# al8n/serf

Measured on NVIDIA H100. Metric: gossip edge-updates/sec @10M nodes, higher is better.
Workload: dtype u32

## Files before the change

### include/serfsim.h

```cpp
#ifndef SERFSIM_H
#define SERFSIM_H

#include <stddef.h>
#include <stdint.h>

#ifdef __cplusplus
extern "C" {
#endif

#define SERFSIM_ABI_VERSION 4u

#define SERFSIM_OK            0
#define SERFSIM_E_INVAL      (-1)
#define SERFSIM_E_NO_DEVICE  (-2)
#define SERFSIM_E_CUDA       (-3)
#define SERFSIM_E_NOMEM      (-4)
#define SERFSIM_E_OVERFLOW   (-5)
#define SERFSIM_E_COMM       (-6)

#define SERFSIM_STATUS_NONE     0u
#define SERFSIM_STATUS_ALIVE    1u
#define SERFSIM_STATUS_LEAVING  2u
#define SERFSIM_STATUS_LEFT     3u
#define SERFSIM_STATUS_FAILED   4u
// ... 122 lines not shown

int serfsim_set_user_events(serfsim_t* h, uint32_t n_events, const uint32_t* content_ids );
int serfsim_event_time       (serfsim_t* h, uint64_t* out );
int serfsim_user_event_seen  (serfsim_t* h, uint32_t event, uint8_t* out );
int serfsim_user_event_ltime (serfsim_t* h, uint32_t event, uint64_t* ltime);
int serfsim_user_event_records(serfsim_t* h, void* out );
int serfsim_user_event_stats (serfsim_t* h, serfsim_uevent_stats_t* out);

int serfsim_set_byzantine  (serfsim_t* h, uint32_t n, const uint32_t* ids , uint32_t delta);
int serfsim_anomaly_flags  (serfsim_t* h, uint8_t* out );
int serfsim_byzantine_stats(serfsim_t* h, serfsim_byz_stats_t* out);

int serfsim_last_step_device_ms(serfsim_t* h, double* ms, uint64_t* kernel_launches);
int serfsim_set_tick_timing(serfsim_t* h, int enabled);
int serfsim_tick_times(serfsim_t* h, uint32_t first_tick, uint32_t n, float* ms_out);

size_t serfsim_comm_blob_size(void);
int    serfsim_comm_export (serfsim_t* h, void* blob);
int    serfsim_comm_connect(serfsim_t* h, const void* blobs );
typedef void (*serfsim_barrier_fn)(void* user);
typedef void (*serfsim_allreduce_u64_fn)(void* user, uint64_t* buf, uint32_t n);
int    serfsim_comm_set_hooks(serfsim_t* h, serfsim_barrier_fn barrier, serfsim_allreduce_u64_fn allreduce, void* user);
int    serfsim_comm_loopback(serfsim_t* h);

#define SERFSIM_WIRE_LEAVE     1u
#define SERFSIM_WIRE_JOIN      2u
#define SERFSIM_WIRE_PUSH_PULL 3u
typedef struct { uint32_t type , prune ; uint64_t ltime, id; } serfsim_wire_intent_t;
typedef struct {
  uint64_t ltime, event_ltime, query_ltime;
// ... 41 lines not shown
```

### serf_b200/csrc/serfsim.cu

```cuda
#include <algorithm>
#include <cmath>
#include <cstdio>
#include <cstdlib>
#include <cstring>
#include <string>
#include <unordered_set>
#include <vector>

#include "../../include/serfsim.h"
#include "tick_kernel.cuh"
#include "wire.cuh"

using namespace sfs;

namespace {

thread_local std::string g_err;

int fail(int code, const std::string& msg) { g_err = msg; return code; }

#define CU(call)                                                                              \
  do {                                                                                        \
    cudaError_t e_ = (call);                                                                  \
    if (e_ != cudaSuccess)                                                                    \
// ... 71 lines not shown
  const uint4** d_peer_snap_rec = nullptr;
  const u64** d_peer_snap_node = nullptr;
  u8* d_hot[2] = {nullptr, nullptr};
  u8* d_hot_static = nullptr;
  u32* d_node_due = nullptr;
  u32* d_carry = nullptr;
  u32* d_tile_due = nullptr;
  u32* d_sched = nullptr;
  u32 n_tiles = 0;
  u32* d_rowptr = nullptr;
  u32* d_col = nullptr;
  u32 *d_ev_node = nullptr, *d_ev_op = nullptr, *d_ev_slot = nullptr;
  size_t ev_cap = 0;
  u64* d_trace = nullptr;
  u32* d_kinds = nullptr;
  u32* d_ones = nullptr;
  u32 trace_cap = 0;
  u32* d_overflow = nullptr;
  u32* pin_overflow = nullptr;
  u32* d_subj = nullptr;
  u64* d_scratch = nullptr;
  void* d_stage = nullptr;
  UeTable ue_table{};
  uint4* d_ue_state = nullptr;
  u32* d_ue_inbox[2] = {nullptr, nullptr};
  u32* d_ue_ltime = nullptr;
  wire::UeWire ue_wire{};
  u8* d_ue_entries = nullptr;
  u64* d_ue_totals = nullptr;
  u32 ue_injected = 0;
// ... 67 lines not shown
  std::vector<cudaEvent_t> tick_ev;
  std::vector<cudaEvent_t> mid_ev;
};

namespace {

int slot_of(const serfsim* h, u32 node) {
  for (u32 s = 0; s < h->R; ++s) if (h->subj[s] == node) return (int)s;
  return -1;
}

int ensure_trace(serfsim* h, u32 need) {
  if (need <= h->trace_cap) return 0;
  u32 cap = std::max<u32>(1024, h->trace_cap);
  while (cap < need) cap *= 2;
  u64* nt = nullptr; u32* nk = nullptr; u64* ng = nullptr;
  const bool sharded = h->cfg.world_size > 1;
  CU(cudaMalloc(&nt, (size_t)cap * 8 * sizeof(u64)));
  CU(cudaMalloc(&nk, ((size_t)cap + 1) * 4 * sizeof(u32)));
  CU(cudaMemsetAsync(nt, 0, (size_t)cap * 8 * sizeof(u64), h->stream));
  CU(cudaMemsetAsync(nk, 0, ((size_t)cap + 1) * 4 * sizeof(u32), h->stream));
  if (sharded) { CU(cudaMalloc(&ng, (size_t)cap * 8 * sizeof(u64))); CU(cudaMemsetAsync(ng, 0, (size_t)cap * 8 * sizeof(u64), h->stream)); }
  if (h->d_trace) {
    CU(cudaMemcpyAsync(nt, h->d_trace, (size_t)h->trace_cap * 8 * sizeof(u64), cudaMemcpyDeviceToDevice, h->stream));
    CU(cudaMemcpyAsync(nk, h->d_kinds, ((size_t)h->trace_cap + 1) * 4 * sizeof(u32), cudaMemcpyDeviceToDevice, h->stream));
    if (sharded) CU(cudaMemcpyAsync(ng, h->d_grow, (size_t)h->trace_cap * 8 * sizeof(u64), cudaMemcpyDeviceToDevice, h->stream));
    CU(cudaStreamSynchronize(h->stream));
    cudaFree(h->d_trace); cudaFree(h->d_kinds); cudaFree(h->d_grow);
  }
  h->d_trace = nt; h->d_kinds = nk; h->d_grow = ng; h->trace_cap = cap;
  return 0;
}

int upload_ops(serfsim* h) {
  if (!h->ops_dirty) return 0;
  std::stable_sort(h->ops.begin(), h->ops.end(), [](const HostOp& a, const HostOp& b) { return a.tick != b.tick ? a.tick < b.tick : a.seq < b.seq; });
  const size_t n = h->ops.size();
  if (n > h->ev_cap) {
    size_t cap = std::max<size_t>(1024, h->ev_cap);
    while (cap < n) cap *= 2;
    if (h->d_ev_node) { cudaFree(h->d_ev_node); cudaFree(h->d_ev_op); cudaFree(h->d_ev_slot); }
    CU(cudaMalloc(&h->d_ev_node, cap * 4)); CU(cudaMalloc(&h->d_ev_op, cap * 4)); CU(cudaMalloc(&h->d_ev_slot, cap * 4));
    h->ev_cap = cap;
  }
  if (n) {
    std::vector<u32> a(n), b(n), c(n);
    for (size_t i = 0; i < n; ++i) { a[i] = h->ops[i].node; b[i] = h->ops[i].op; c[i] = h->ops[i].slot; }
    CU(cudaMemcpyAsync(h->d_ev_node, a.data(), n * 4, cudaMemcpyHostToDevice, h->stream));
    CU(cudaMemcpyAsync(h->d_ev_op, b.data(), n * 4, cudaMemcpyHostToDevice, h->stream));
    CU(cudaMemcpyAsync(h->d_ev_slot, c.data(), n * 4, cudaMemcpyHostToDevice, h->stream));
    CU(cudaStreamSynchronize(h->stream));
  }
  h->ops_dirty = false;
  return 0;
}

bool future_ops(const serfsim* h, u32 after_tick) {
  return !h->ops.empty() && h->ops.back().tick > after_tick;
}

int launch_ticks(serfsim* h, u32 n) {
  if (!h->has_topo) return fail(SERFSIM_E_INVAL, "serfsim_step: no topology set");
  if (h->cfg.world_size > 1 && !h->connected) return fail(SERFSIM_E_COMM, "serfsim_step: world_size > 1 but serfsim_comm_connect was not called");
  int rc = upload_ops(h);
  if (rc) return rc;
  rc = ensure_trace(h, h->tick + n + 1);
  if (rc) return rc;
  if (!h->timing_open) { CU(cudaEventRecord(h->ev0, h->stream)); h->timing_open = true; h->last_launches = 0; h->launch_log.clear(); h->launch_log_first = h->tick; }
  const bool sharded = h->cfg.world_size > 1;
  const u64* grow = sharded ? h->d_grow : h->d_trace;
  for (u32 i = 0; i < n; ++i) {
    const u32 t = h->tick;
    const u64 launches_before = h->last_launches;
// ... 10 lines not shown
    p.fanout = h->cfg.fanout; p.probe_every = h->cfg.probe_interval_ticks; p.tick = t;
    p.down_mask = (~h->up_mask) & ((1u << h->R) - 1);
    h->ever_down |= p.down_mask;
    p.seed_lo = (u32)h->cfg.seed; p.seed_hi = (u32)(h->cfg.seed >> 32); p.ev_begin = eb; p.ev_end = ee;
    p.rules = h->rules;
    for (u32 s = 0; s < h->R; ++s) p.subj[s] = h->subj[s];
    p.rec = h->d_rec; p.qword = h->d_qword; p.inbox_rd = h->d_inbox[(t & 1) ^ 1]; p.inbox_wr = h->d_inbox[t & 1];
    p.node_state = h->d_node; p.busy = h->d_busy; p.watch = h->d_watch; p.row_ptr = h->d_rowptr; p.col = h->d_col;
    p.ev_node = h->d_ev_node; p.ev_op = h->d_ev_op; p.ev_slot = h->d_ev_slot;
    p.row = h->d_trace + (size_t)t * 8;
    p.kinds_prev = h->d_kinds + (size_t)t * 4;
    p.kinds_cur = h->d_kinds + ((size_t)t + 1) * 4;
    p.overflow = h->d_overflow;
    p.hot_rd = h->d_hot[(t & 1) ^ 1]; p.hot_wr = h->d_hot[t & 1];
    p.stage_col_bytes = h->stage_col_bytes;
    p.reap_now = (h->cfg.reap_interval_ticks && ((t + 1) % h->cfg.reap_interval_ticks) == 0) ? 1u : 0u;
    p.tombstone_ticks = h->cfg.tombstone_timeout_ticks; p.reconnect_ticks = h->cfg.reconnect_timeout_ticks; p.intent_ticks = h->cfg.recent_intent_timeout_ticks;
    p.stride = h->stride; p.n_tiles = h->n_tiles; p.tiles_per_cta = (h->n_tiles + h->grid - 1) / h->grid;
    p.force_all = (h->cfg.trace != 0) || h->no_skip || p.reap_now;
    p.compact = h->compact ? 1u : 0u;
    p.dedup = h->dedup ? 1u : 0u;
    p.udeg = h->udeg; p.ahead = h->ahead;
    p.tile_due = h->d_tile_due; p.node_due = h->d_node_due; p.hot_static = h->d_hot_static; p.sched = h->d_sched;
    p.sleep_on = (h->no_skip || h->byz_on) ? 0u : 1u;
    p.pp_every = (u32)std::max(0, h->cfg.push_pull_interval_ticks); p.reap_every = h->cfg.reap_interval_ticks;
    p.host_idle_until = h->d_pin_ctl + 2;
    const u32 xpar = h->xepoch & 1;
    p.world = (u32)h->cfg.world_size; p.rank = (u32)h->cfg.rank; p.shard_size = h->shard_size; p.win_cap = h->win_cap;
    p.win_data = h->d_peer_data[xpar]; p.send_count = h->d_send_count;
    p.peer_ctrl = h->d_peer_ctrl; p.stamp = h->xepoch + 1; p.xpar = xpar; p.loopback = h->loopback ? 1u : 0u;
    p.fuse_publish = (sharded && !h->byz_on && !getenv("SERFSIM_NO_FUSE")) ? 1u : 0u;
// ... 23 lines not shown
    if (h->ue_table.n) {
      UeParams u{};
      u.n_local = h->count; u.first = h->first; u.n_global = h->N; u.R = h->R; u.fanout = h->cfg.fanout; u.tick = t;
      u.seed_lo = p.seed_lo; u.seed_hi = p.seed_hi; u.limit = h->rules.limit; u.ev_begin = eb; u.ev_end = ee;
      u.table = h->ue_table; u.state = h->d_ue_state; u.inbox_rd = h->d_ue_inbox[(t & 1) ^ 1]; u.inbox_wr = h->d_ue_inbox[t & 1];
      u.ltime = h->d_ue_ltime; u.node_state = h->d_node; u.busy = h->d_busy; u.row_ptr = h->d_rowptr; u.col = h->d_col;
      u.ev_node = h->d_ev_node; u.ev_op = h->d_ev_op; u.ev_slot = h->d_ev_slot;
      u.row = p.row; u.totals = h->d_ue_totals; u.overflow = h->d_overflow; u.sched = h->d_sched;
      u.world = (u32)h->cfg.world_size; u.rank = (u32)h->cfg.rank; u.shard_size = h->shard_size; u.win_cap = h->win_cap;
      u.win_data = h->d_peer_data[h->xepoch & 1]; u.send_count = h->d_send_count;
      u.gate = gate; u.gate.evaluate = 1u;
      launch_uevent(u, h->cfg.trace != 0, h->stream);
      h->last_launches++;
    }
    const bool sv_ok = h->sv && h->R > 1 && h->R < 32 && !h->cfg.trace && p.sleep_on && !h->byz_on;
    const bool pass_tick = sv_ok && !sharded && ee == eb && !p.reap_now && t + 1 < CARRY_TICKS;
    const bool dual = sv_ok && sharded && __builtin_popcount(h->ever_down) == 1;
    if (pass_tick || dual) {
      const bool all = ee > eb || p.reap_now;
      p.views_host = all ? 0xffffffffu : h->ever_down;
      p.sv_mode = h->sv == 2 ? SV_CHECK : SV_GENERAL;
      p.sv_slot = h->ever_down ? (u32)__builtin_ctz(h->ever_down) : 0u; p.sv_R = h->R;
    }
    if (pass_tick && h->sv == 1) {
      p.sv_mode = SV_PASS; p.carry = h->d_carry;
      p.tiles_per_cta = (h->n_tiles + h->grid_sv - 1) / h->grid_sv;
      for (u32 s0 = 0; s0 < h->R; ++s0) {
        TickParams q = p;
        q.gate.evaluate = s0 == 0 ? p.gate.evaluate : 0u; q.sv_wshift = s0; q.sv_slot = s0;
        q.rec = p.rec + 2 * (size_t)s0 * h->stride; q.qword = p.qword + (size_t)s0 * h->stride;
        q.inbox_rd = p.inbox_rd + (size_t)s0 * h->stride; q.inbox_wr = p.inbox_wr + (size_t)s0 * h->stride;
        q.subj[0] = p.subj[s0]; q.down_mask = (p.down_mask >> s0) & 1u;
        launch_tick_pass(q, h->grid_sv, h->stream);
        h->last_launches++;
      }
    } else {
      launch_tick(p, h->cfg.trace != 0, h->grid, h->stream);
      h->last_launches++;
    }
    if (dual && h->sv == 1) {
      TickParams q = p;
      const u32 s0 = p.sv_slot;
      q.sv_mode = SV_SINGLE; q.gate.evaluate = 0u; q.sv_wshift = s0;
      q.rec = p.rec + 2 * (size_t)s0 * h->stride; q.qword = p.qword + (size_t)s0 * h->stride;
// ... 184 lines not shown
  CU(cudaMemsetAsync(h->d_inbox[1], 0, inbox_bytes, h->stream));
  CU(cudaStreamSynchronize(h->stream));
  *(volatile u32*)h->pin_overflow = 0;
  ((volatile u32*)h->pin_ctl)[2] = 0;
  CU(cudaMemsetAsync(h->d_busy, 0, h->stride, h->stream));
  CU(cudaMemsetAsync(h->d_qword, 0, (size_t)h->R * h->stride * 4, h->stream));
  CU(cudaMemsetAsync(h->d_hot[0], 0, h->n_tiles, h->stream));
  CU(cudaMemsetAsync(h->d_hot[1], 0, h->n_tiles, h->stream));
  CU(cudaMemsetAsync(h->d_tile_due, 0xff, (size_t)h->n_tiles * sizeof(u32), h->stream));
  CU(cudaMemsetAsync(h->d_node_due, 0xff, (size_t)h->stride * sizeof(u32), h->stream));
  if (h->d_carry) CU(cudaMemsetAsync(h->d_carry, 0, (size_t)h->stride * sizeof(u32), h->stream));
  CU(cudaMemsetAsync(h->d_sched, 0, SCHED_WORDS * sizeof(u32), h->stream));
  if (h->d_trace) {
    CU(cudaMemsetAsync(h->d_trace, 0, (size_t)h->trace_cap * 8 * sizeof(u64), h->stream));
    CU(cudaMemsetAsync(h->d_kinds, 0, ((size_t)h->trace_cap + 1) * 4 * sizeof(u32), h->stream));
  }
  if (h->d_grow) CU(cudaMemsetAsync(h->d_grow, 0, (size_t)h->trace_cap * 8 * sizeof(u64), h->stream));
  CU(cudaMemsetAsync(h->d_runctl, 0, 2 * sizeof(u32), h->stream));
  if (h->d_send_count) CU(cudaMemsetAsync(h->d_send_count, 0, sizeof(u32) * 8, h->stream));
  { int rc = ue_reset(h); if (rc) return rc; }
  if (h->d_anomaly) { CU(cudaMemsetAsync(h->d_anomaly, 0, h->stride, h->stream)); CU(cudaMemsetAsync(h->d_byz_totals, 0, 4 * 8, h->stream)); }
  { int rc = refresh_watchers(h); if (rc) return rc; }
  CU(cudaStreamSynchronize(h->stream));
  return 0;
}

void free_all(serfsim* h) {
  for (void* p : h->ipc_opened) cudaIpcCloseMemHandle(p);
  for (cudaEvent_t e : h->tick_ev) cudaEventDestroy(e);
  cudaFree(h->d_hot_static); cudaFree(h->d_tile_due); cudaFree(h->d_node_due); cudaFree(h->d_carry); cudaFree(h->d_sched);
  cudaFree(h->d_hot[0]); cudaFree(h->d_hot[1]); cudaFree(h->d_busy); cudaFree(h->d_watch); cudaFree(h->d_snap_rec); cudaFree(h->d_snap_node); cudaFree(h->d_peer_snap_rec); cudaFree(h->d_peer_snap_node);
  cudaFree(h->d_qword);
  cudaFree(h->d_rec); cudaFree(h->d_inbox[0]); cudaFree(h->d_inbox[1]); cudaFree(h->d_node); cudaFree(h->d_rowptr); cudaFree(h->d_col);
  cudaFree(h->d_ev_node); cudaFree(h->d_ev_op); cudaFree(h->d_ev_slot); cudaFree(h->d_trace); cudaFree(h->d_kinds); cudaFree(h->d_ones);
  if (h->pin_overflow) cudaFreeHost(h->pin_overflow);
  cudaFree(h->d_subj); cudaFree(h->d_scratch); cudaFree(h->d_stage);
  cudaFree(h->d_byz_ids); cudaFree(h->d_anomaly); cudaFree(h->d_byz_totals); cudaFree(h->d_peer_anomaly);
  cudaFree(h->d_ue_snap); cudaFree(h->d_peer_ue_snap);
  cudaFree(h->d_ue_entries);
  cudaFree(h->d_ue_state); cudaFree(h->d_ue_inbox[0]); cudaFree(h->d_ue_inbox[1]); cudaFree(h->d_ue_ltime); cudaFree(h->d_ue_totals);
  for (int par = 0; par < 2; ++par) { cudaFree(h->d_win_data[par]); cudaFree(h->d_peer_data[par]); }
  cudaFree(h->d_ctrl); cudaFree(h->d_send_count); cudaFree(h->d_peer_ctrl);
  for (auto& b : h->res) { cudaFree(b.d); if (b.copied) cudaEventDestroy(b.copied); }
  if (h->ev_extracted) cudaEventDestroy(h->ev_extracted);
  if (h->copy_stream) cudaStreamDestroy(h->copy_stream);
  if (h->pin_ctl) cudaFreeHost(h->pin_ctl);
  cudaFree(h->d_runctl); cudaFree(h->d_grow);
  if (h->ev0) cudaEventDestroy(h->ev0);
  if (h->ev1) cudaEventDestroy(h->ev1);
// ... 703 lines not shown
}

int serfsim_set_tick_timing(serfsim_t* h, int enabled) {
  if (!h) return fail(SERFSIM_E_INVAL, "null handle");
  h->tick_timing = enabled != 0;
  return 0;
}

int serfsim_tick_times(serfsim_t* h, uint32_t first_tick, uint32_t n, float* ms_out) {
  if (!h || !ms_out) return fail(SERFSIM_E_INVAL, "null argument");
  if (((size_t)first_tick + n) * 2 > h->tick_ev.size()) return fail(SERFSIM_E_INVAL, "tick timing was not enabled for that range");
  CU(cudaStreamSynchronize(h->stream));
  for (u32 i = 0; i < n; ++i) CU(cudaEventElapsedTime(ms_out + i, h->tick_ev[2 * ((size_t)first_tick + i)], h->tick_ev[2 * ((size_t)first_tick + i) + 1]));
  return 0;
}

struct comm_blob { cudaIpcMemHandle_t data[2]; cudaIpcMemHandle_t ctrl; cudaIpcMemHandle_t snap_rec, snap_node, anomaly, ue_snap; u32 win_cap; u32 rank; u32 has_snap; u32 has_ue_snap; unsigned char dev_uuid[16]; };

size_t serfsim_comm_blob_size(void) { return sizeof(comm_blob); }

int serfsim_comm_export(serfsim_t* h, void* blob) {
  if (!h || !blob) return fail(SERFSIM_E_INVAL, "null argument");
  if (h->cfg.world_size < 2) return fail(SERFSIM_E_INVAL, "world_size == 1: nothing to export");
  comm_blob b{};
  for (int par = 0; par < 2; ++par) CU(cudaIpcGetMemHandle(&b.data[par], h->d_win_data[par]));
  CU(cudaIpcGetMemHandle(&b.ctrl, h->d_ctrl));
  CU(cudaIpcGetMemHandle(&b.anomaly, h->d_anomaly));
  if (h->d_ue_snap) { CU(cudaIpcGetMemHandle(&b.ue_snap, h->d_ue_snap)); b.has_ue_snap = 1; }
  b.win_cap = h->win_cap; b.rank = (u32)h->cfg.rank;
#ifndef SERFSIM_EMU
// ... 102 lines not shown
```

### serf_b200/csrc/tick_kernel.cu

```cuda
#include <cstdlib>

#include "tick_kernel.cuh"
#include "byz.cuh"

namespace sfs {

namespace {

constexpr int BLOCK = 256;
#ifndef SFS_MB_R1
#define SFS_MB_R1 3
#endif
#ifndef SFS_MB_R1S
#define SFS_MB_R1S SFS_MB_R1
#endif
#ifndef SFS_MB_RN
#define SFS_MB_RN 1
#endif
constexpr u32 TILE_SHIFT = 8;
constexpr u32 MAX_TILES_PER_CTA = 1024;
static_assert((1u << TILE_SHIFT) == BLOCK, "tile = block");

struct Words { u32 w[8]; };

// ... 278 lines not shown
  x.mL = x.mJ = x.mM = x.qw = 0; x.any = 0; x.mailmask = 0; x.qmask = 0;
  for (u32 s2 = 0; s2 < s_hi; ++s2) {
    const u32 l = kL ? ld_u32_stream(p.inbox_rd + (size_t)(KIND_LEAVE * R + s2) * nl + vl, pol_first) : 0u;
    const u32 j = kJ ? ld_u32_stream(p.inbox_rd + (size_t)(KIND_JOIN * R + s2) * nl + vl, pol_first) : 0u;
    const u32 m = kM ? ld_u32_stream(p.inbox_rd + (size_t)(KIND_ML * R + s2) * nl + vl, pol_first) : 0u;
    const u32 q = p.qword[(size_t)s2 * nl + vl];
    SFS_COUNT(6, 4);
    if (R1 || s2 == x.keep) { x.mL = l; x.mJ = j; x.mM = m; x.qw = q; }
    x.any |= l | j | m;
    x.mailmask |= ((l | j | m) ? 1u : 0u) << s2;
    x.qmask |= (q ? 1u : 0u) << s2;
  }
  if (PASS) x.any |= x.qw | ((due && (carry_of(p, vl) & CARRY_TDUE)) ? 1u : 0u);
  return x;
}
__device__ __forceinline__ bool node_active(const TickParams& p, const Pre& x, bool due) {
  return (x.busy & 7u) != 0 || x.any != 0 || p.reap_now != 0 || (due && (x.busy & 8u) && x.nd <= p.tick);
}

template <int FMAX>
struct Ahead { u64 ns; Words rec; u32 cand[FMAX]; u32 valid; };

__device__ __forceinline__ u32 sleeping_deadline(const Pre& x, bool due) { return (due && (x.busy & 8u)) ? x.nd : NO_DEADLINE; }

#if defined(SFS_COLD_INLINE)
#define SFS_COLD __forceinline__
#elif defined(SERFSIM_EMU)
#define SFS_COLD __attribute__((noinline))
#else
#define SFS_COLD __noinline__
#endif
__device__ SFS_COLD void cold_host_op(Rec& r, u32& clock, u32& sstate, u32 op, bool op_here, bool self, bool up_r, u32 limit) {
// ... 88 lines not shown
      cur = ld_rec256(p.rec + 2 * (size_t)vl, pol_first);
    }
    merge_q(cur, pre.qw);
  };
  if (upfront) { load_node(); load_rec0(); }
  const u32 busy = pre.busy;
  u32 mL = pre.mL, mJ = pre.mJ, mM = pre.mM;
  if (STAGED) { mL = kL ? sv.inL[lt] : 0u; mJ = kJ ? sv.inJ[lt] : 0u; mM = kM ? sv.inM[lt] : 0u; }

  u32 nd = pre.nd;
  if (R1 && due && (busy & 8u)) nd = p.node_due[vl];
  const u32 sleeping = (due && (busy & 8u)) ? nd : NO_DEADLINE;
  bool timers_due = sleeping <= p.tick;
  u32 cr = 0;
  if (PASS && due) { cr = carry_of(p, vl); if (cr & CARRY_SEEN) timers_due = (cr & CARRY_TDUE) != 0; }
  if (!TRACE && !STAGED && !((busy & 7u) != 0 || pre.any != 0 || p.reap_now != 0 || timers_due)) { mind = min(mind, sleeping); if (due && (busy & 8u)) SFS_PROBE(20); return false; }
  if (PASS && !due) cr = carry_of(p, vl);
  if (STAGED && !TRACE && !((busy & 7u) || (mL | mJ | mM) || p.reap_now || timers_due)) { mind = min(mind, sleeping); return false; }
#define SFS_WMASK() ((busy & 4u) ? ((u32)p.watch[vl] >> p.sv_wshift) : 0u)
  const bool ahead = !R1 && !STAGED && ah.valid;
  if (ahead) { ns = ah.ns; row0 = vl * p.udeg; row1 = row0 + p.udeg; }
  else if (!upfront) { load_node(); if (R1) load_rec0(); }

  u32 clock = (u32)ns;
  const bool up_r = (ns & NS_UP) != 0;
  u32 sstate = (u32)(ns >> 40) & 3;
  const u32 deg = row1 - row0;

  u32 op = 0, op_slot = 0;
  if (busy & 2) { u32 slot_tmp = 0; op = cold_find_op(p, v, slot_tmp); op_slot = slot_tmp; }
  bool up_s = up_r;
// ... 235 lines not shown
#pragma unroll
  for (int i = 0; i < 8; ++i) {
    const u32 s = warp_sum((u32)vals[i]);
    if (lane == 0) red[i][wid] = s;
  }
  u64 hs = 0;
  if (TRACE) hs = warp_sum64(c.hash);
  __syncthreads();
  if (threadIdx.x == 0 && dsusp_cta) atomicAdd(reinterpret_cast<unsigned long long*>(p.sched + SCHED_SUSPECTS), (unsigned long long)(long long)dsusp_cta);
  if (threadIdx.x < 8) {
    u64 s = 0;
#pragma unroll
    for (int w = 0; w < BLOCK / 32; ++w) s += red[threadIdx.x][w];
    if (s) {
      if (threadIdx.x < 5) atomicAdd((unsigned long long*)(p.row + threadIdx.x), (unsigned long long)s);
      else atomicAdd(p.kinds_cur + (threadIdx.x - 5), (u32)min(s, (u64)0xffffffffu));
    }
  }
  if (TRACE && lane == 0 && hs) atomicAdd((unsigned long long*)(p.row + 7), (unsigned long long)hs);
  { const u32 vw = __reduce_or_sync(0xffffffffu, c.views); if (lane == 0 && vw) atomicOr(p.sched + SCHED_VIEWS_NEXT, vw); }
  if (PASS && p.sv_slot + 1u < p.sv_R) return;
  __threadfence();
  __syncthreads();
  if (threadIdx.x == 0) last_s = (atomicAdd(p.sched + SCHED_TICKET, 1u) == gridDim.x - 1) ? 1u : 0u;
  __syncthreads();
  if (!last_s) return;
  __threadfence();
  volatile u32* sched = p.sched;
  volatile u64* row = p.row;
  const u64 suspects = *reinterpret_cast<volatile u64*>(p.sched + SCHED_SUSPECTS);
  __shared__ u32 quiet_s;
// ... 51 lines not shown
    const u32 views = (sv_base | p.views_host) & ((1u << p.sv_R) - 1u);
    work = (views >> p.sv_slot) & 1u;
    carry_out = (views >> p.sv_slot) > 1u;
    if (work) SFS_PROBE(21);
    else if (p.sv_slot != 0 && p.sv_slot + 1u < p.sv_R) return;
  } else if (p.sv_mode != SV_OFF) {
    const u32 sv_base = p.tick >= p.sched[SCHED_VIEWS_FROM] ? p.sched[SCHED_VIEWS_NEW] : p.sched[SCHED_VIEWS_OLD];
    const u32 views = (sv_base | p.views_host) & ((1u << p.sv_R) - 1u);
    const bool single = views == (1u << p.sv_slot);
    if (p.sv_mode == SV_SINGLE) { if (!single) return; SFS_PROBE(21); }
    else if (p.sv_mode == SV_GENERAL && single) return;
    if (p.sv_mode == SV_CHECK && (single || p.world == 1)) sv_views = views;
  }
  if (threadIdx.x == 0) dsusp_s = 0;
  Counters c = {};
  const bool kL = p.kinds_prev[KIND_LEAVE] != 0, kJ = p.kinds_prev[KIND_JOIN] != 0, kM = p.kinds_prev[KIND_ML] != 0;
  const u64 pol_first = policy_evict_first(), pol_last = policy_evict_last();
  const int lane = threadIdx.x & 31;
  if (SHARDED && threadIdx.x < (BLOCK / 32) * MAX_WORLD) xs->cnt[threadIdx.x / MAX_WORLD][threadIdx.x % MAX_WORLD] = 0;
  bool wrote_remote = false;
  u32 resv = 0, rlen = 0;

  const u32 prev_msgs = p.kinds_prev[KIND_LEAVE] + p.kinds_prev[KIND_JOIN] + p.kinds_prev[KIND_ML];
  const bool dense_now = prev_msgs >= (p.n_tiles >> 1) + 1;
  const bool all_hot = p.force_all || p.kinds_prev[3] != 0;
  const bool mark = !dense_now;
  const bool saturated = prev_msgs >= (p.n_local >> 1);
  if (dense_now && blockIdx.x == 0 && threadIdx.x == 0) p.kinds_cur[3] = 1;

  const u32 tile0 = blockIdx.x * p.tiles_per_cta;
  const u32 ntile = tile0 < p.n_tiles ? min(p.tiles_per_cta, p.n_tiles - tile0) : 0;
  if (SHARDED && saturated && ntile && (u32)lane < p.world && (u32)lane != p.rank) { resv = atomicAdd(p.send_count + lane, XW_FLUSH); rlen = XW_FLUSH; }
  if (PASS && p.sv_slot != 0) tile_decisions(p, hot_s, tile0, ntile, p.sv_slot + 1u == p.sv_R, work); else scan_tiles(p, hot_s, tile0, ntile, all_hot, PASS);
  __syncthreads();
  if (PASS && !work && p.sv_slot + 1u < p.sv_R) return;
  constexpr u32 GROUP = SHARDED ? 4 : 8;
  __shared__ uint4 act_s[GROUP * BLOCK];
  __shared__ u32 act_n;
  __shared__ u8 pend_s[GROUP];
  __shared__ u16 gt_s[GROUP];
  const bool compact = !TRACE && !saturated && !p.reap_now && p.compact;
  if (compact) {
    u32 i = 0;
// ... 6 lines not shown
      __syncthreads();
      Pre pr[GROUP];
#pragma unroll
      for (u32 g = 0; g < GROUP; ++g) {
        pr[g] = Pre{};
        if (g < ng) {
          const u32 vn = ((tile0 + gt_s[g]) << TILE_SHIFT) + threadIdx.x;
          if (vn < p.n_local) pr[g] = prefetch_node<R1, PASS>(p, vn, kL, kJ, kM, pol_first, PASS && (hot_s[gt_s[g]] & 2u) != 0);
        }
      }
#pragma unroll
      for (u32 g = 0; g < GROUP; ++g) {
        const bool due_g = g < ng && (hot_s[gt_s[g]] & 2u) != 0;
        Pre prg = pr[g];
        if (due_g && (prg.busy & 8u)) prg.nd = p.node_due[((tile0 + gt_s[g]) << TILE_SHIFT) + threadIdx.x];
        const bool act = g < ng && node_active(p, prg, due_g);
        if (due_g) {
          const u32 wm = warp_min(act ? NO_DEADLINE : sleeping_deadline(prg, true));
          if (lane == 0 && wm != NO_DEADLINE) atomicMin(p.tile_due + tile0 + gt_s[g], wm);
          if (!act && (prg.busy & 8u)) SFS_PROBE(20);
        }
        const u32 bal = __ballot_sync(0xffffffffu, act);
        if (bal) {
          u32 base = 0;
          if (lane == 0) base = atomicAdd(&act_n, (u32)__popc(bal));
          base = __shfl_sync(0xffffffffu, base, 0);
          if (act) act_s[base + (u32)__popc(bal & ((1u << lane) - 1u))] =
              make_uint4((g << 8) | threadIdx.x | (pr[g].busy << 16) | ((pr[g].any ? 1u : 0u) << 24), pr[g].mL, pr[g].mJ, pr[g].mM);
        }
      }
      __syncthreads();
// ... 632 lines not shown
```

### serf_b200/csrc/tick_kernel.cuh

```cuda
#pragma once
#include <cuda_runtime.h>

#include "record.cuh"
#include "uevent.cuh"

#if defined(SERFSIM_EMU) && defined(__CUDACC__)
#error "SERFSIM_EMU is the host-only test build of tests/emu (g++); the product is built by nvcc without it"
#endif
#ifndef SERFSIM_EMU
#define SFS_LAUNCH(grid, block, smem, stream, ...) __VA_ARGS__<<<(grid), (block), (smem), (stream)>>>
constexpr int SFS_SMS = 132;
#else
constexpr int SFS_SMS = 1;
#endif
#ifdef SERFSIM_EMU
#define SFS_PROBE(i) (emu::probes[i]++)
#define SFS_COUNT(i, n) (emu::probes[i] += (n))
#else
#define SFS_PROBE(i) ((void)0)
#define SFS_COUNT(i, n) ((void)0)
#endif

namespace sfs {

// ... 60 lines not shown
  Gate gate;
  u32 udeg;
  u32* tile_due;
  u32* node_due;
  const u8* hot_static;
  u32* sched;
  u32 sleep_on;
  u32 pp_every, reap_every;
  u32* const* peer_ctrl; u32 stamp, xpar, loopback, fuse_publish;
  u32 shard_inv, xcap;
  u32 sv_wshift;
  u32 sv_mode, views_host, sv_slot, sv_R;
  u32 ahead;
  u32* host_idle_until;
  u32* carry;
};
constexpr u32 SCHED_TICKET = 0, SCHED_IDLE_UNTIL = 1, SCHED_UE_ACTIVITY = 2, SCHED_AWAKE = 3, SCHED_SUSPECTS = 4 ,
              SCHED_LOCAL_QUIET = 6, SCHED_LOCAL_UNTIL = 7 ,
              SCHED_VIEWS_NEW = 8 , SCHED_VIEWS_NEXT = 9 ,
              SCHED_VIEWS_OLD = 10 , SCHED_VIEWS_FROM = 11, SCHED_WORDS = 12;
constexpr u32 SV_OFF = 0, SV_GENERAL = 1, SV_SINGLE = 2, SV_CHECK = 3, SV_PASS = 4;
constexpr u32 CARRY_PK = 0xfu, CARRY_AWAKE = 0x10u, CARRY_TDUE = 0x20u, CARRY_SEEN = 0x40u, CARRY_TICKS = 1u << 24;
constexpr u32 NO_DEADLINE = 0xffffffffu;
__device__ __forceinline__ bool tick_is_idle(const u32* sched, u32 tick, u32 ev_begin, u32 ev_end) {
  return sched && ev_begin == ev_end && tick < sched[SCHED_IDLE_UNTIL];
}

constexpr u32 CTRL_U32 = 2 * 16;
constexpr u32 CTRL_SUMS_OFF = CTRL_U32 * 4;
constexpr u32 CTRL_FIELDS = 11;
// ... 104 lines not shown
```

### serf_b200/sim.py

```python
import ctypes as C
import enum
import os

import numpy as np

_HERE = os.path.dirname(os.path.abspath(__file__))
ABI_VERSION = 4


class MemberStatus(enum.IntEnum):
    NONE = 0
    ALIVE = 1
    LEAVING = 2
    LEFT = 3
    FAILED = 4


class MlState(enum.IntEnum):
    ALIVE = 0
    SUSPECT = 1
    DEAD = 2
    LEFT = 3


# ... 94 lines not shown
    "user_event_ltime": (C.c_int, [_vp, _u32, C.POINTER(_u64)]),
    "user_event_records": (C.c_int, [_vp, _vp]),
    "user_event_stats": (C.c_int, [_vp, C.POINTER(UserEventStats)]),
}
PRODUCT_ONLY = {
    "serfsim_abi_version": (_u32, []),
    "serfsim_default_config": (None, [C.POINTER(Config)]),
    "serfsim_last_error": (C.c_char_p, []),
    "serfsim_shard_range": (C.c_int, [_vp, C.POINTER(_u32), C.POINTER(_u32)]),
    "serfsim_set_event_cb": (C.c_int, [_vp, EVENT_CB, _vp]),
    "serfsim_results_async": (C.c_int, [_vp, _u32, _vp, _vp, _vp]),
    "serfsim_results_wait": (C.c_int, [_vp]),
    "serfsim_last_step_device_ms": (C.c_int, [_vp, C.POINTER(C.c_double), C.POINTER(_u64)]),
    "serfsim_set_tick_timing": (C.c_int, [_vp, C.c_int]),
    "serfsim_tick_times": (C.c_int, [_vp, _u32, _u32, _vp]),
    "serfsim_comm_blob_size": (C.c_size_t, []),
    "serfsim_comm_export": (C.c_int, [_vp, _vp]),
    "serfsim_comm_connect": (C.c_int, [_vp, _vp]),
    "serfsim_comm_set_hooks": (C.c_int, [_vp, BARRIER_FN, ALLREDUCE_FN, _vp]),
    "serfsim_comm_loopback": (C.c_int, [_vp]),
    "serfsim_set_user_event_content": (C.c_int, [_vp, _u32, _vp, _vp, _vp, _vp]),
    "serfsim_wire_local_state_range": (C.c_int, [_vp, _u32, _u32, _vp, C.c_size_t, _vp, C.POINTER(C.c_size_t)]),
    "serfsim_wire_decode_events_batch": (C.c_int, [_vp, _vp, _vp, _u32, _vp, _vp, _vp]),
}

_LIB = None


def library_path():
    return os.environ.get("SERFSIM_LIB") or os.path.join(_HERE, "libserfsim.so")
# ... 227 lines not shown
        ms, n = C.c_double(), _u64()
        self._check(self._lib.serfsim_last_step_device_ms(self._h, C.byref(ms), C.byref(n)))
        return ms.value, n.value

    def set_tick_timing(self, enabled=True):
        self._check(self._lib.serfsim_set_tick_timing(self._h, int(enabled)))

    def tick_times_ms(self, first=0, n=None):
        if n is None:
            n = self.stats()["tick"] - first
        out = np.zeros(n, dtype=np.float32)
        if n:
            self._check(self._lib.serfsim_tick_times(self._h, int(first), int(n), out.ctypes.data))
        return out

    def set_event_callback(self, fn):
        def tramp(_user, tick, ty, ids, n):
            fn(tick, ty, [ids[i] for i in range(n)])
        cb = EVENT_CB(tramp)
        self._keep.append(cb)
        self._check(self._lib.serfsim_set_event_cb(self._h, cb, None))

    def connect(self, all_gather_bytes, barrier, allreduce_u64):
        def _bar(_u):
            barrier()

        def _ar(_u, buf, n):
            arr = np.ctypeslib.as_array(buf, shape=(n,))
            allreduce_u64(arr)
        b, a = BARRIER_FN(_bar), ALLREDUCE_FN(_ar)
# ... 64 lines not shown
```

Before: 21.04 billion.

## Track per-view message kinds in pass mode to gate work per slot

In per-slot pass mode, each view launch now keeps its own leave/join/ML kind counters in a new device buffer. The next tick reads these per-view counters instead of the global ones to decide which message kinds to process and whether the view is saturated. Node activity in pass mode also ignores the lowest busy bit, so fewer nodes are woken. The change adds extra atomics, allocation and probes, a debug accessor API, and risks correctness if the per-view gating misses messages.

```diff
diff --git a/include/serfsim.h b/include/serfsim.h
--- a/include/serfsim.h
+++ b/include/serfsim.h
@@ -160,6 +160,7 @@
 int serfsim_last_step_device_ms(serfsim_t* h, double* ms, uint64_t* kernel_launches);
 int serfsim_set_tick_timing(serfsim_t* h, int enabled);
 int serfsim_tick_times(serfsim_t* h, uint32_t first_tick, uint32_t n, float* ms_out);
+int serfsim_tick_view_kinds(serfsim_t* h, uint32_t first_tick, uint32_t n, uint32_t* out);
 
 size_t serfsim_comm_blob_size(void);
 int    serfsim_comm_export (serfsim_t* h, void* blob);
diff --git a/serf_b200/csrc/serfsim.cu b/serf_b200/csrc/serfsim.cu
--- a/serf_b200/csrc/serfsim.cu
+++ b/serf_b200/csrc/serfsim.cu
@@ -109,6 +109,7 @@
   size_t ev_cap = 0;
   u64* d_trace = nullptr;
   u32* d_kinds = nullptr;
+  u32* d_view_kinds = nullptr;
   u32* d_ones = nullptr;
   u32 trace_cap = 0;
   u32* d_overflow = nullptr;
@@ -206,21 +207,24 @@
   if (need <= h->trace_cap) return 0;
   u32 cap = std::max<u32>(1024, h->trace_cap);
   while (cap < need) cap *= 2;
-  u64* nt = nullptr; u32* nk = nullptr; u64* ng = nullptr;
+  u64* nt = nullptr; u32* nk = nullptr; u32* nv = nullptr; u64* ng = nullptr;
   const bool sharded = h->cfg.world_size > 1;
   CU(cudaMalloc(&nt, (size_t)cap * 8 * sizeof(u64)));
   CU(cudaMalloc(&nk, ((size_t)cap + 1) * 4 * sizeof(u32)));
+  CU(cudaMalloc(&nv, ((size_t)cap + 1) * h->R * 4 * sizeof(u32)));
   CU(cudaMemsetAsync(nt, 0, (size_t)cap * 8 * sizeof(u64), h->stream));
   CU(cudaMemsetAsync(nk, 0, ((size_t)cap + 1) * 4 * sizeof(u32), h->stream));
+  CU(cudaMemsetAsync(nv, 0, ((size_t)cap + 1) * h->R * 4 * sizeof(u32), h->stream));
   if (sharded) { CU(cudaMalloc(&ng, (size_t)cap * 8 * sizeof(u64))); CU(cudaMemsetAsync(ng, 0, (size_t)cap * 8 * sizeof(u64), h->stream)); }
   if (h->d_trace) {
     CU(cudaMemcpyAsync(nt, h->d_trace, (size_t)h->trace_cap * 8 * sizeof(u64), cudaMemcpyDeviceToDevice, h->stream));
     CU(cudaMemcpyAsync(nk, h->d_kinds, ((size_t)h->trace_cap + 1) * 4 * sizeof(u32), cudaMemcpyDeviceToDevice, h->stream));
+    CU(cudaMemcpyAsync(nv, h->d_view_kinds, ((size_t)h->trace_cap + 1) * h->R * 4 * sizeof(u32), cudaMemcpyDeviceToDevice, h->stream));
     if (sharded) CU(cudaMemcpyAsync(ng, h->d_grow, (size_t)h->trace_cap * 8 * sizeof(u64), cudaMemcpyDeviceToDevice, h->stream));
     CU(cudaStreamSynchronize(h->stream));
-    cudaFree(h->d_trace); cudaFree(h->d_kinds); cudaFree(h->d_grow);
-  }
-  h->d_trace = nt; h->d_kinds = nk; h->d_grow = ng; h->trace_cap = cap;
+    cudaFree(h->d_trace); cudaFree(h->d_kinds); cudaFree(h->d_view_kinds); cudaFree(h->d_grow);
+  }
+  h->d_trace = nt; h->d_kinds = nk; h->d_view_kinds = nv; h->d_grow = ng; h->trace_cap = cap;
   return 0;
 }
 
@@ -249,6 +253,21 @@
 
 bool future_ops(const serfsim* h, u32 after_tick) {
   return !h->ops.empty() && h->ops.back().tick > after_tick;
+}
+
+bool ops_at(const serfsim* h, u32 t) {
+  auto it = std::lower_bound(h->ops.begin(), h->ops.end(), t, [](const HostOp& o, u32 tt) { return o.tick < tt; });
+  return it != h->ops.end() && it->tick == t;
+}
+bool reap_tick(const serfsim* h, u32 t) { return h->cfg.reap_interval_ticks && ((t + 1) % h->cfg.reap_interval_ticks) == 0; }
+bool pass_tick(const serfsim* h, u32 t, u32 mode) {
+  const bool sleep_on = !h->no_skip && !h->byz_on;
+  return h->sv == mode && h->R > 1 && h->R < 32 && !h->cfg.trace && sleep_on && h->cfg.world_size == 1 && !ops_at(h, t) && !reap_tick(h, t) &&
+         t + 1 < CARRY_TICKS;
+}
+bool view_kinds_valid(const serfsim* h, u32 t) {
+  const u32 pp = (u32)std::max(0, h->cfg.push_pull_interval_ticks);
+  return pass_tick(h, t, 1) && !(pp && (t + 1) % pp == 0);
 }
 
 int launch_ticks(serfsim* h, u32 n) {
@@ -289,7 +308,7 @@
     p.overflow = h->d_overflow;
     p.hot_rd = h->d_hot[(t & 1) ^ 1]; p.hot_wr = h->d_hot[t & 1];
     p.stage_col_bytes = h->stage_col_bytes;
-    p.reap_now = (h->cfg.reap_interval_ticks && ((t + 1) % h->cfg.reap_interval_ticks) == 0) ? 1u : 0u;
+    p.reap_now = reap_tick(h, t) ? 1u : 0u;
     p.tombstone_ticks = h->cfg.tombstone_timeout_ticks; p.reconnect_ticks = h->cfg.reconnect_timeout_ticks; p.intent_ticks = h->cfg.recent_intent_timeout_ticks;
     p.stride = h->stride; p.n_tiles = h->n_tiles; p.tiles_per_cta = (h->n_tiles + h->grid - 1) / h->grid;
     p.force_all = (h->cfg.trace != 0) || h->no_skip || p.reap_now;
@@ -343,20 +362,23 @@
       h->last_launches++;
     }
     const bool sv_ok = h->sv && h->R > 1 && h->R < 32 && !h->cfg.trace && p.sleep_on && !h->byz_on;
-    const bool pass_tick = sv_ok && !sharded && ee == eb && !p.reap_now && t + 1 < CARRY_TICKS;
+    const bool passes = pass_tick(h, t, 1), check = pass_tick(h, t, 2);
     const bool dual = sv_ok && sharded && __builtin_popcount(h->ever_down) == 1;
-    if (pass_tick || dual) {
+    if (passes || check || dual) {
       const bool all = ee > eb || p.reap_now;
       p.views_host = all ? 0xffffffffu : h->ever_down;
       p.sv_mode = h->sv == 2 ? SV_CHECK : SV_GENERAL;
       p.sv_slot = h->ever_down ? (u32)__builtin_ctz(h->ever_down) : 0u; p.sv_R = h->R;
     }
-    if (pass_tick && h->sv == 1) {
+    if (passes) {
       p.sv_mode = SV_PASS; p.carry = h->d_carry;
       p.tiles_per_cta = (h->n_tiles + h->grid_sv - 1) / h->grid_sv;
+      const bool own = t > 0 && view_kinds_valid(h, t - 1);
       for (u32 s0 = 0; s0 < h->R; ++s0) {
         TickParams q = p;
         q.gate.evaluate = s0 == 0 ? p.gate.evaluate : 0u; q.sv_wshift = s0; q.sv_slot = s0;
+        q.view_kinds_prev = own ? h->d_view_kinds + ((size_t)t * h->R + s0) * 4 : p.kinds_prev;
+        q.view_kinds_cur = h->d_view_kinds + (((size_t)t + 1) * h->R + s0) * 4;
         q.rec = p.rec + 2 * (size_t)s0 * h->stride; q.qword = p.qword + (size_t)s0 * h->stride;
         q.inbox_rd = p.inbox_rd + (size_t)s0 * h->stride; q.inbox_wr = p.inbox_wr + (size_t)s0 * h->stride;
         q.subj[0] = p.subj[s0]; q.down_mask = (p.down_mask >> s0) & 1u;
@@ -571,6 +593,7 @@
   if (h->d_trace) {
     CU(cudaMemsetAsync(h->d_trace, 0, (size_t)h->trace_cap * 8 * sizeof(u64), h->stream));
     CU(cudaMemsetAsync(h->d_kinds, 0, ((size_t)h->trace_cap + 1) * 4 * sizeof(u32), h->stream));
+    CU(cudaMemsetAsync(h->d_view_kinds, 0, ((size_t)h->trace_cap + 1) * h->R * 4 * sizeof(u32), h->stream));
   }
   if (h->d_grow) CU(cudaMemsetAsync(h->d_grow, 0, (size_t)h->trace_cap * 8 * sizeof(u64), h->stream));
   CU(cudaMemsetAsync(h->d_runctl, 0, 2 * sizeof(u32), h->stream));
@@ -589,7 +612,7 @@
   cudaFree(h->d_hot[0]); cudaFree(h->d_hot[1]); cudaFree(h->d_busy); cudaFree(h->d_watch); cudaFree(h->d_snap_rec); cudaFree(h->d_snap_node); cudaFree(h->d_peer_snap_rec); cudaFree(h->d_peer_snap_node);
   cudaFree(h->d_qword);
   cudaFree(h->d_rec); cudaFree(h->d_inbox[0]); cudaFree(h->d_inbox[1]); cudaFree(h->d_node); cudaFree(h->d_rowptr); cudaFree(h->d_col);
-  cudaFree(h->d_ev_node); cudaFree(h->d_ev_op); cudaFree(h->d_ev_slot); cudaFree(h->d_trace); cudaFree(h->d_kinds); cudaFree(h->d_ones);
+  cudaFree(h->d_ev_node); cudaFree(h->d_ev_op); cudaFree(h->d_ev_slot); cudaFree(h->d_trace); cudaFree(h->d_kinds); cudaFree(h->d_view_kinds); cudaFree(h->d_ones);
   if (h->pin_overflow) cudaFreeHost(h->pin_overflow);
   cudaFree(h->d_subj); cudaFree(h->d_scratch); cudaFree(h->d_stage);
   cudaFree(h->d_byz_ids); cudaFree(h->d_anomaly); cudaFree(h->d_byz_totals); cudaFree(h->d_peer_anomaly);
@@ -1323,6 +1346,17 @@
   for (u32 i = 0; i < n; ++i) CU(cudaEventElapsedTime(ms_out + i, h->tick_ev[2 * ((size_t)first_tick + i)], h->tick_ev[2 * ((size_t)first_tick + i) + 1]));
   return 0;
 }
+int serfsim_tick_view_kinds(serfsim_t* h, uint32_t first_tick, uint32_t n, uint32_t* out) {
+  if (!h || !out) return fail(SERFSIM_E_INVAL, "null argument");
+  if ((size_t)first_tick + n > h->tick) return fail(SERFSIM_E_INVAL, "ticks not run yet");
+  if (!n) return 0;
+  std::vector<u32> rows((size_t)n * h->R * 4);
+  CU(cudaMemcpyAsync(rows.data(), h->d_view_kinds + ((size_t)first_tick + 1) * h->R * 4, rows.size() * sizeof(u32), cudaMemcpyDeviceToHost, h->stream));
+  CU(cudaStreamSynchronize(h->stream));
+  for (size_t i = 0; i < (size_t)n * h->R; ++i)
+    for (u32 k = 0; k < 3; ++k) out[i * 3 + k] = rows[i * 4 + k];
+  return 0;
+}
 
 struct comm_blob { cudaIpcMemHandle_t data[2]; cudaIpcMemHandle_t ctrl; cudaIpcMemHandle_t snap_rec, snap_node, anomaly, ue_snap; u32 win_cap; u32 rank; u32 has_snap; u32 has_ue_snap; unsigned char dev_uuid[16]; };
 
diff --git a/serf_b200/csrc/tick_kernel.cu b/serf_b200/csrc/tick_kernel.cu
--- a/serf_b200/csrc/tick_kernel.cu
+++ b/serf_b200/csrc/tick_kernel.cu
@@ -316,8 +316,11 @@
   if (PASS) x.any |= x.qw | ((due && (carry_of(p, vl) & CARRY_TDUE)) ? 1u : 0u);
   return x;
 }
+template <bool PASS = false>
+__device__ __forceinline__ u32 busy_business(u32 busy) { return busy & (PASS ? 6u : 7u); }
+template <bool PASS = false>
 __device__ __forceinline__ bool node_active(const TickParams& p, const Pre& x, bool due) {
-  return (x.busy & 7u) != 0 || x.any != 0 || p.reap_now != 0 || (due && (x.busy & 8u) && x.nd <= p.tick);
+  return busy_business<PASS>(x.busy) != 0 || x.any != 0 || p.reap_now != 0 || (due && (x.busy & 8u) && x.nd <= p.tick);
 }
 
 template <int FMAX>
@@ -436,7 +439,7 @@
   bool timers_due = sleeping <= p.tick;
   u32 cr = 0;
   if (PASS && due) { cr = carry_of(p, vl); if (cr & CARRY_SEEN) timers_due = (cr & CARRY_TDUE) != 0; }
-  if (!TRACE && !STAGED && !((busy & 7u) != 0 || pre.any != 0 || p.reap_now != 0 || timers_due)) { mind = min(mind, sleeping); if (due && (busy & 8u)) SFS_PROBE(20); return false; }
+  if (!TRACE && !STAGED && !(busy_business<PASS>(busy) != 0 || pre.any != 0 || p.reap_now != 0 || timers_due)) { mind = min(mind, sleeping); if (due && (busy & 8u)) SFS_PROBE(20); return false; }
   if (PASS && !due) cr = carry_of(p, vl);
   if (STAGED && !TRACE && !((busy & 7u) || (mL | mJ | mM) || p.reap_now || timers_due)) { mind = min(mind, sleeping); return false; }
 #define SFS_WMASK() ((busy & 4u) ? ((u32)p.watch[vl] >> p.sv_wshift) : 0u)
@@ -702,7 +705,10 @@
     for (int w = 0; w < BLOCK / 32; ++w) s += red[threadIdx.x][w];
     if (s) {
       if (threadIdx.x < 5) atomicAdd((unsigned long long*)(p.row + threadIdx.x), (unsigned long long)s);
-      else atomicAdd(p.kinds_cur + (threadIdx.x - 5), (u32)min(s, (u64)0xffffffffu));
+      else {
+        atomicAdd(p.kinds_cur + (threadIdx.x - 5), (u32)min(s, (u64)0xffffffffu));
+        if (PASS) atomicAdd(p.view_kinds_cur + (threadIdx.x - 5), (u32)min(s, (u64)0xffffffffu));
+      }
     }
   }
   if (TRACE && lane == 0 && hs) atomicAdd((unsigned long long*)(p.row + 7), (unsigned long long)hs);
@@ -784,7 +790,8 @@
   }
   if (threadIdx.x == 0) dsusp_s = 0;
   Counters c = {};
-  const bool kL = p.kinds_prev[KIND_LEAVE] != 0, kJ = p.kinds_prev[KIND_JOIN] != 0, kM = p.kinds_prev[KIND_ML] != 0;
+  const u32* const kv = PASS ? p.view_kinds_prev : p.kinds_prev;
+  const bool kL = kv[KIND_LEAVE] != 0, kJ = kv[KIND_JOIN] != 0, kM = kv[KIND_ML] != 0;
   const u64 pol_first = policy_evict_first(), pol_last = policy_evict_last();
   const int lane = threadIdx.x & 31;
   if (SHARDED && threadIdx.x < (BLOCK / 32) * MAX_WORLD) xs->cnt[threadIdx.x / MAX_WORLD][threadIdx.x % MAX_WORLD] = 0;
@@ -795,8 +802,14 @@
   const bool dense_now = prev_msgs >= (p.n_tiles >> 1) + 1;
   const bool all_hot = p.force_all || p.kinds_prev[3] != 0;
   const bool mark = !dense_now;
-  const bool saturated = prev_msgs >= (p.n_local >> 1);
+  const u32 own_msgs = PASS ? kv[KIND_LEAVE] + kv[KIND_JOIN] + kv[KIND_ML] : prev_msgs;
+  const bool saturated = own_msgs >= (p.n_local >> 1);
   if (dense_now && blockIdx.x == 0 && threadIdx.x == 0) p.kinds_cur[3] = 1;
+  if (PASS && work && threadIdx.x == 0) {
+    if (kv == p.kinds_prev) SFS_PROBE(23);
+    if (!saturated && prev_msgs >= (p.n_local >> 1) && p.compact) SFS_PROBE(24);
+    if ((!kL && p.kinds_prev[KIND_LEAVE]) || (!kJ && p.kinds_prev[KIND_JOIN]) || (!kM && p.kinds_prev[KIND_ML])) SFS_PROBE(25);
+  }
 
   const u32 tile0 = blockIdx.x * p.tiles_per_cta;
   const u32 ntile = tile0 < p.n_tiles ? min(p.tiles_per_cta, p.n_tiles - tile0) : 0;
@@ -833,7 +846,7 @@
         const bool due_g = g < ng && (hot_s[gt_s[g]] & 2u) != 0;
         Pre prg = pr[g];
         if (due_g && (prg.busy & 8u)) prg.nd = p.node_due[((tile0 + gt_s[g]) << TILE_SHIFT) + threadIdx.x];
-        const bool act = g < ng && node_active(p, prg, due_g);
+        const bool act = g < ng && node_active<PASS>(p, prg, due_g);
         if (due_g) {
           const u32 wm = warp_min(act ? NO_DEADLINE : sleeping_deadline(prg, true));
           if (lane == 0 && wm != NO_DEADLINE) atomicMin(p.tile_due + tile0 + gt_s[g], wm);
diff --git a/serf_b200/csrc/tick_kernel.cuh b/serf_b200/csrc/tick_kernel.cuh
--- a/serf_b200/csrc/tick_kernel.cuh
+++ b/serf_b200/csrc/tick_kernel.cuh
@@ -98,6 +98,7 @@
   u32 ahead;
   u32* host_idle_until;
   u32* carry;
+  const u32* view_kinds_prev; u32* view_kinds_cur;
 };
 constexpr u32 SCHED_TICKET = 0, SCHED_IDLE_UNTIL = 1, SCHED_UE_ACTIVITY = 2, SCHED_AWAKE = 3, SCHED_SUSPECTS = 4 ,
               SCHED_LOCAL_QUIET = 6, SCHED_LOCAL_UNTIL = 7 ,
diff --git a/serf_b200/sim.py b/serf_b200/sim.py
--- a/serf_b200/sim.py
+++ b/serf_b200/sim.py
@@ -132,6 +132,7 @@
     "serfsim_last_step_device_ms": (C.c_int, [_vp, C.POINTER(C.c_double), C.POINTER(_u64)]),
     "serfsim_set_tick_timing": (C.c_int, [_vp, C.c_int]),
     "serfsim_tick_times": (C.c_int, [_vp, _u32, _u32, _vp]),
+    "serfsim_tick_view_kinds": (C.c_int, [_vp, _u32, _u32, _vp]),
     "serfsim_comm_blob_size": (C.c_size_t, []),
     "serfsim_comm_export": (C.c_int, [_vp, _vp]),
     "serfsim_comm_connect": (C.c_int, [_vp, _vp]),
@@ -389,6 +390,14 @@
             self._check(self._lib.serfsim_tick_times(self._h, int(first), int(n), out.ctypes.data))
         return out
 
+    def tick_view_kinds(self, first=0, n=None):
+        if n is None:
+            n = self.stats()["tick"] - first
+        out = np.zeros((n, self.slots, 3), dtype=np.uint32)
+        if n:
+            self._check(self._lib.serfsim_tick_view_kinds(self._h, int(first), int(n), out.ctypes.data))
+        return out
+
     def set_event_callback(self, fn):
         def tramp(_user, tick, ty, ids, n):
             fn(tick, ty, [ids[i] for i in range(n)])
```

Result: faster. 21.88 billion, median of 6 (+4.0%).
